# SobeyMIL/MVOC

Measured on AMD Instinct MI355X. Metric: UNet3D denoising steps/sec, 16x512^2 frames, inversion+compose, higher is better.
Workload: dtype f16

## Files before the change

mvoc_amd/csrc/pnp.hip:

```cpp
#include "common.h"

namespace {

struct PnpArgs {
  half_t* x[2];
  const half_t* masks;
  long chunk_stride, f_stride, p_stride;
  int nobj, frames, height, width, channels, mask_h, mask_w, base_chunk0;
  int ndst;
  float sy, sx;
  long total;
  int nsrc;
  unsigned obj_map;
};

template <bool MAPPED>
__device__ __forceinline__ int obj_chunk(const PnpArgs& p, int j) {
  if constexpr (MAPPED) return (int)((p.obj_map >> (4 * j)) & 15u);
  return j + 1;
}

template <bool MAPPED>
__device__ __forceinline__ int chunk_count(const PnpArgs& p) {
  if constexpr (MAPPED) return p.nsrc + p.ndst;
  return p.nobj + 1 + p.ndst;
}

__device__ __forceinline__ float blend16(float inj, float obj, float m) {
  const float om = r16(1.0f - m);
  return r16(r16(inj * om) + r16(obj * m));
}

__device__ __forceinline__ int nearest_src(int dst, float scale, int in_size) {
  return min((int)floorf(dst * scale), in_size - 1);
}

template <bool MAPPED>
__global__ __launch_bounds__(256) void pnp_tokens_kernel(const PnpArgs p) {
  const long idx = (long)blockIdx.x * 256 + threadIdx.x;
  if (idx >= p.total) return;
// ... 557 lines not shown
  MVOC_REQUIRE(d->nobj >= 1 && d->nobj <= 4, -2, "pnp: nobj %d not in [1,4]", d->nobj);
  MVOC_REQUIRE(d->frames > 0 && d->height > 0 && d->width > 0 && d->channels > 0 && d->mask_h > 0 && d->mask_w > 0, -1,
               "pnp: bad dims");
  a.x[0] = (half_t*)d->x;
  a.x[1] = (half_t*)d->x2;
  a.masks = (const half_t*)d->masks;
  a.chunk_stride = d->chunk_stride; a.f_stride = d->f_stride; a.p_stride = d->p_stride;
  a.nobj = d->nobj; a.frames = d->frames; a.height = d->height; a.width = d->width; a.channels = d->channels;
  a.mask_h = d->mask_h; a.mask_w = d->mask_w; a.base_chunk0 = d->base_chunk0;
  MVOC_REQUIRE(d->ndst >= 0 && d->ndst <= 2, -1, "pnp: ndst %d not in {0 (= 2), 1, 2}", d->ndst);
  a.ndst = d->ndst == 0 ? 2 : d->ndst;
  a.sy = (float)d->mask_h / (float)d->height;
  a.sx = (float)d->mask_w / (float)d->width;
  a.nsrc = d->nobj + 1;
  a.obj_map = 0;
  return 0;
}

int fill_map(const mvoc_pnp_desc* d, int32_t nsrc, const int32_t* obj_chunk_host, PnpArgs& a, int& nread) {
  MVOC_REQUIRE(obj_chunk_host, -1, "pnp mapped: null obj_chunk");
  MVOC_REQUIRE(nsrc >= 1 && nsrc <= d->nobj + 1, -1, "pnp mapped: nsrc %d not in [1, nobj + 1 = %d]", nsrc, d->nobj + 1);
  unsigned map = 0, seen = d->base_chunk0 ? 1u : 0u;
  for (int j = 0; j < d->nobj; ++j) {
    const int c = obj_chunk_host[j];
    MVOC_REQUIRE(c >= 0 && c < nsrc, -1, "pnp mapped: obj_chunk[%d] = %d not in [0, nsrc = %d)", j, c, nsrc);
    map |= (unsigned)c << (4 * j);
    seen |= 1u << c;
  }
  a.nsrc = nsrc;
  a.obj_map = map;
// ... 127 lines not shown
  return 0;
}

template <int NOBJ>
void launch_nchw_variants_n(bool vec, dim3 grid, hipStream_t s, const PnpArgs& a, int nvar) {
  if (vec)
    hipLaunchKernelGGL((pnp_nchw_variants_kernel<8, NOBJ>), grid, dim3(256), 0, s, a, nvar);
  else
    hipLaunchKernelGGL((pnp_nchw_variants_kernel<1, NOBJ>), grid, dim3(256), 0, s, a, nvar);
}

}

extern "C" int mvoc_pnp_blend_scatter_tokens_variants(const mvoc_pnp_desc* d, int32_t nsrc, const int32_t* obj_chunk,
                                                      int32_t nvar, void* stream) {
  PnpArgs a;
  double chunks = 0;
  if (int rc = fill_variants(d, nsrc, obj_chunk, nvar, a, chunks)) return rc;
  MVOC_REQUIRE(d->channels % 8 == 0 && d->chunk_stride % 8 == 0 && d->f_stride % 8 == 0 && d->p_stride % 8 == 0, -2,
               "pnp tokens: channels/strides must be multiples of 8");
  a.total = (long)d->frames * d->height * d->width * (d->channels / 8);
  const long nblk = (a.total + 255) / 256;
  MVOC_REQUIRE(nblk < 0x7fffffffL, -2, "pnp tokens: grid too large");
  const int ntens = d->x2 ? 2 : 1;
  hipStream_t s = (hipStream_t)stream;
  const double elems = (double)d->frames * d->height * d->width * d->channels;
  MvocProfScope prof(MVOC_FAM_PNP, s, ntens * (elems * 2.0 * chunks + 2.0 * d->nobj * d->frames * d->height * d->width));
  const dim3 grid((unsigned)nblk, ntens);
  switch (d->nobj) {
    case 1: hipLaunchKernelGGL(pnp_tokens_variants_kernel<1>, grid, dim3(256), 0, s, a, (int)nvar); break;
    case 2: hipLaunchKernelGGL(pnp_tokens_variants_kernel<2>, grid, dim3(256), 0, s, a, (int)nvar); break;
    case 3: hipLaunchKernelGGL(pnp_tokens_variants_kernel<3>, grid, dim3(256), 0, s, a, (int)nvar); break;
    default: hipLaunchKernelGGL(pnp_tokens_variants_kernel<4>, grid, dim3(256), 0, s, a, (int)nvar); break;
  }
  return mvoc_check_launch("pnp_tokens_variants_kernel");
}

extern "C" int mvoc_pnp_blend_scatter_nchw_variants(const mvoc_pnp_desc* d, int32_t nsrc, const int32_t* obj_chunk,
                                                    int32_t nvar, void* stream) {
  PnpArgs a;
  double chunks = 0;
  if (int rc = fill_variants(d, nsrc, obj_chunk, nvar, a, chunks)) return rc;
  const long hw = (long)d->height * d->width;
  const bool vec = hw % 8 == 0;
  a.total = (long)d->frames * d->channels * (vec ? hw / 8 : hw);
  const long nblk = (a.total + 255) / 256;
  MVOC_REQUIRE(nblk < 0x7fffffffL, -2, "pnp nchw: grid too large");
  const int ntens = d->x2 ? 2 : 1;
  hipStream_t s = (hipStream_t)stream;
  const double elems = (double)d->frames * hw * d->channels;
  MvocProfScope prof(MVOC_FAM_PNP, s, ntens * (elems * 2.0 * chunks + 2.0 * d->nobj * d->frames * hw));
  const dim3 grid((unsigned)nblk, ntens);
  switch (d->nobj) {
    case 1: launch_nchw_variants_n<1>(vec, grid, s, a, nvar); break;
// ... 19 lines not shown
  return 0;
}

template <int NOBJ>
void launch_nchw_variants_sel_n(bool vec, dim3 grid, hipStream_t s, const PnpArgs& a, int nvar, unsigned active) {
  if (vec)
    hipLaunchKernelGGL((pnp_nchw_variants_sel_kernel<8, NOBJ>), grid, dim3(256), 0, s, a, nvar, active);
  else
    hipLaunchKernelGGL((pnp_nchw_variants_sel_kernel<1, NOBJ>), grid, dim3(256), 0, s, a, nvar, active);
}

}

extern "C" int mvoc_pnp_blend_scatter_tokens_variants_sel(const mvoc_pnp_desc* d, int32_t nsrc, const int32_t* obj_chunk,
                                                          int32_t nvar, uint32_t active, void* stream) {
  PnpArgs a;
  double chunks = 0;
  if (int rc = fill_variants_sel(d, nsrc, obj_chunk, nvar, active, a, chunks)) return rc;
  MVOC_REQUIRE(d->channels % 8 == 0 && d->chunk_stride % 8 == 0 && d->f_stride % 8 == 0 && d->p_stride % 8 == 0, -2,
               "pnp tokens: channels/strides must be multiples of 8");
  a.total = (long)d->frames * d->height * d->width * (d->channels / 8);
  const long nblk = (a.total + 255) / 256;
  MVOC_REQUIRE(nblk < 0x7fffffffL, -2, "pnp tokens: grid too large");
  const int ntens = d->x2 ? 2 : 1;
  hipStream_t s = (hipStream_t)stream;
  const double elems = (double)d->frames * d->height * d->width * d->channels;
  MvocProfScope prof(MVOC_FAM_PNP, s, ntens * (elems * 2.0 * chunks + 2.0 * d->nobj * d->frames * d->height * d->width));
  const dim3 grid((unsigned)nblk, ntens);
  const unsigned act = active;
  switch (d->nobj) {
    case 1: hipLaunchKernelGGL(pnp_tokens_variants_sel_kernel<1>, grid, dim3(256), 0, s, a, (int)nvar, act); break;
    case 2: hipLaunchKernelGGL(pnp_tokens_variants_sel_kernel<2>, grid, dim3(256), 0, s, a, (int)nvar, act); break;
    case 3: hipLaunchKernelGGL(pnp_tokens_variants_sel_kernel<3>, grid, dim3(256), 0, s, a, (int)nvar, act); break;
    default: hipLaunchKernelGGL(pnp_tokens_variants_sel_kernel<4>, grid, dim3(256), 0, s, a, (int)nvar, act); break;
  }
  return mvoc_check_launch("pnp_tokens_variants_sel_kernel");
}

extern "C" int mvoc_pnp_blend_scatter_nchw_variants_sel(const mvoc_pnp_desc* d, int32_t nsrc, const int32_t* obj_chunk,
                                                        int32_t nvar, uint32_t active, void* stream) {
  PnpArgs a;
  double chunks = 0;
  if (int rc = fill_variants_sel(d, nsrc, obj_chunk, nvar, active, a, chunks)) return rc;
  const long hw = (long)d->height * d->width;
  const bool vec = hw % 8 == 0;
  a.total = (long)d->frames * d->channels * (vec ? hw / 8 : hw);
  const long nblk = (a.total + 255) / 256;
  MVOC_REQUIRE(nblk < 0x7fffffffL, -2, "pnp nchw: grid too large");
  const int ntens = d->x2 ? 2 : 1;
  hipStream_t s = (hipStream_t)stream;
  const double elems = (double)d->frames * hw * d->channels;
  MvocProfScope prof(MVOC_FAM_PNP, s, ntens * (elems * 2.0 * chunks + 2.0 * d->nobj * d->frames * hw));
  const dim3 grid((unsigned)nblk, ntens);
  switch (d->nobj) {
    case 1: launch_nchw_variants_sel_n<1>(vec, grid, s, a, nvar, active); break;
// ... 12 lines not shown
  return fill_variants_sel(d, nsrc, obj_chunk, nvar, active, a, chunks);
}

template <int NOBJ>
void launch_nchw_placed_n(bool vec, dim3 grid, hipStream_t s, const PnpArgs& a, int nvar, unsigned active, const int* place) {
  if (vec)
    hipLaunchKernelGGL((pnp_nchw_placed_kernel<8, NOBJ>), grid, dim3(256), 0, s, a, nvar, active, place);
  else
    hipLaunchKernelGGL((pnp_nchw_placed_kernel<1, NOBJ>), grid, dim3(256), 0, s, a, nvar, active, place);
}

}

extern "C" int mvoc_pnp_blend_scatter_tokens_placed(const mvoc_pnp_desc* d, int32_t nsrc, const int32_t* obj_chunk, int32_t nvar,
                                                    uint32_t active, const int32_t* place, void* stream) {
  PnpArgs a;
  double chunks = 0;
  if (int rc = fill_placed(d, nsrc, obj_chunk, nvar, active, place, a, chunks)) return rc;
  MVOC_REQUIRE(d->channels % 8 == 0 && d->chunk_stride % 8 == 0 && d->f_stride % 8 == 0 && d->p_stride % 8 == 0, -2,
               "pnp tokens: channels/strides must be multiples of 8");
  a.total = (long)d->frames * d->height * d->width * (d->channels / 8);
  const long nblk = (a.total + 255) / 256;
  MVOC_REQUIRE(nblk < 0x7fffffffL, -2, "pnp tokens: grid too large");
  const int ntens = d->x2 ? 2 : 1;
  hipStream_t s = (hipStream_t)stream;
  const double elems = (double)d->frames * d->height * d->width * d->channels;
  MvocProfScope prof(MVOC_FAM_PNP, s, ntens * (elems * 2.0 * chunks + 2.0 * d->nobj * d->frames * d->height * d->width));
  const dim3 grid((unsigned)nblk, ntens);
  const unsigned act = active;
  const int* pl = (const int*)place;
  switch (d->nobj) {
    case 1: hipLaunchKernelGGL(pnp_tokens_placed_kernel<1>, grid, dim3(256), 0, s, a, (int)nvar, act, pl); break;
    case 2: hipLaunchKernelGGL(pnp_tokens_placed_kernel<2>, grid, dim3(256), 0, s, a, (int)nvar, act, pl); break;
    case 3: hipLaunchKernelGGL(pnp_tokens_placed_kernel<3>, grid, dim3(256), 0, s, a, (int)nvar, act, pl); break;
    default: hipLaunchKernelGGL(pnp_tokens_placed_kernel<4>, grid, dim3(256), 0, s, a, (int)nvar, act, pl); break;
  }
  return mvoc_check_launch("pnp_tokens_placed_kernel");
}

extern "C" int mvoc_pnp_blend_scatter_nchw_placed(const mvoc_pnp_desc* d, int32_t nsrc, const int32_t* obj_chunk, int32_t nvar,
                                                  uint32_t active, const int32_t* place, void* stream) {
  PnpArgs a;
  double chunks = 0;
  if (int rc = fill_placed(d, nsrc, obj_chunk, nvar, active, place, a, chunks)) return rc;
  const long hw = (long)d->height * d->width;
  const bool vec = hw % 8 == 0;
  a.total = (long)d->frames * d->channels * (vec ? hw / 8 : hw);
  const long nblk = (a.total + 255) / 256;
  MVOC_REQUIRE(nblk < 0x7fffffffL, -2, "pnp nchw: grid too large");
  const int ntens = d->x2 ? 2 : 1;
  hipStream_t s = (hipStream_t)stream;
  const double elems = (double)d->frames * hw * d->channels;
  MvocProfScope prof(MVOC_FAM_PNP, s, ntens * (elems * 2.0 * chunks + 2.0 * d->nobj * d->frames * hw));
  const dim3 grid((unsigned)nblk, ntens);
  const int* pl = (const int*)place;
  switch (d->nobj) {
// ... 19 lines not shown
}

template <int NOBJ>
void launch_nchw_placed_variants_n(bool vec, dim3 grid, hipStream_t s, const PnpArgs& a, int nvar, unsigned active,
                                   const int* place) {
  if (vec)
    hipLaunchKernelGGL((pnp_nchw_placed_variants_kernel<8, NOBJ>), grid, dim3(256), 0, s, a, nvar, active, place);
  else
    hipLaunchKernelGGL((pnp_nchw_placed_variants_kernel<1, NOBJ>), grid, dim3(256), 0, s, a, nvar, active, place);
}

}

extern "C" int mvoc_pnp_blend_scatter_tokens_placed_variants(const mvoc_pnp_desc* d, int32_t nsrc, const int32_t* obj_chunk,
                                                             int32_t nvar, uint32_t active, const int32_t* place, void* stream) {
  PnpArgs a;
  double chunks = 0;
  int on = 0;
  if (int rc = fill_placed_variants(d, nsrc, obj_chunk, nvar, active, place, a, chunks, on)) return rc;
  MVOC_REQUIRE(d->channels % 8 == 0 && d->chunk_stride % 8 == 0 && d->f_stride % 8 == 0 && d->p_stride % 8 == 0, -2,
               "pnp tokens: channels/strides must be multiples of 8");
  a.total = (long)d->frames * d->height * d->width * (d->channels / 8);
  const long nblk = (a.total + 255) / 256;
  MVOC_REQUIRE(nblk < 0x7fffffffL, -2, "pnp tokens: grid too large");
  const int ntens = d->x2 ? 2 : 1;
  hipStream_t s = (hipStream_t)stream;
  const double elems = (double)d->frames * d->height * d->width * d->channels;
  MvocProfScope prof(MVOC_FAM_PNP, s,
                     ntens * (elems * 2.0 * chunks + 2.0 * on * d->nobj * d->frames * d->height * d->width) +
                         8.0 * nvar * d->nobj * d->frames);
  const dim3 grid((unsigned)nblk, ntens);
  const unsigned act = active;
  const int* pl = (const int*)place;
  switch (d->nobj) {
    case 1: hipLaunchKernelGGL(pnp_tokens_placed_variants_kernel<1>, grid, dim3(256), 0, s, a, (int)nvar, act, pl); break;
    case 2: hipLaunchKernelGGL(pnp_tokens_placed_variants_kernel<2>, grid, dim3(256), 0, s, a, (int)nvar, act, pl); break;
    case 3: hipLaunchKernelGGL(pnp_tokens_placed_variants_kernel<3>, grid, dim3(256), 0, s, a, (int)nvar, act, pl); break;
    default: hipLaunchKernelGGL(pnp_tokens_placed_variants_kernel<4>, grid, dim3(256), 0, s, a, (int)nvar, act, pl); break;
  }
  return mvoc_check_launch("pnp_tokens_placed_variants_kernel");
}

extern "C" int mvoc_pnp_blend_scatter_nchw_placed_variants(const mvoc_pnp_desc* d, int32_t nsrc, const int32_t* obj_chunk,
                                                           int32_t nvar, uint32_t active, const int32_t* place, void* stream) {
  PnpArgs a;
  double chunks = 0;
  int on = 0;
  if (int rc = fill_placed_variants(d, nsrc, obj_chunk, nvar, active, place, a, chunks, on)) return rc;
  const long hw = (long)d->height * d->width;
  const bool vec = hw % 8 == 0;
  a.total = (long)d->frames * d->channels * (vec ? hw / 8 : hw);
  const long nblk = (a.total + 255) / 256;
  MVOC_REQUIRE(nblk < 0x7fffffffL, -2, "pnp nchw: grid too large");
  const int ntens = d->x2 ? 2 : 1;
  hipStream_t s = (hipStream_t)stream;
  const double elems = (double)d->frames * hw * d->channels;
  MvocProfScope prof(MVOC_FAM_PNP, s,
                     ntens * (elems * 2.0 * chunks + 2.0 * on * d->nobj * d->frames * hw) + 8.0 * nvar * d->nobj * d->frames);
  const dim3 grid((unsigned)nblk, ntens);
// ... 40 lines not shown
  MVOC_REQUIRE(latents && bg && objs && masks && out && n_per > 0 && nobj >= 0, -1, "latent_fusion_variants: null operand / empty");
  MVOC_REQUIRE(nvar >= 1 && nvar <= 8, -1, "latent_fusion_variants: nvar %d not in [1, 8]", nvar);
  hipStream_t s = (hipStream_t)stream;
  const long n = (long)n_per * nvar;
  MvocProfScope prof(MVOC_FAM_MISC, s, 2.0 * n * 2 + 2.0 * n_per * (1 + 2 * nobj));
  const float mix = (float)mix_ratio, omix = (float)(1.0 - mix_ratio);
  hipLaunchKernelGGL(fusion_variants_kernel, dim3((unsigned)((n + 255) / 256)), dim3(256), 0, s, (const half_t*)latents,
                     (const half_t*)bg, (const half_t*)objs, (const half_t*)masks, (half_t*)out, nobj, (long)n_per, n, mix, omix,
                     obj_random_noise_fusion);
  return mvoc_check_launch("fusion_variants_kernel");
}

extern "C" int mvoc_pnp_blend_scatter_tokens(const mvoc_pnp_desc* d, void* stream) {
  PnpArgs a;
  if (int rc = fill_args(d, a)) return rc;
  return launch_tokens<false>(d, a, d->nobj + 1, stream);
}

extern "C" int mvoc_pnp_blend_scatter_nchw(const mvoc_pnp_desc* d, void* stream) {
  PnpArgs a;
  if (int rc = fill_args(d, a)) return rc;
  return launch_nchw<false>(d, a, d->nobj + 1, stream);
}

extern "C" int mvoc_pnp_blend_scatter_tokens_mapped(const mvoc_pnp_desc* d, int32_t nsrc, const int32_t* obj_chunk,
                                                    void* stream) {
  PnpArgs a;
  int nread = 0;
  if (int rc = fill_args(d, a)) return rc;
  if (int rc = fill_map(d, nsrc, obj_chunk, a, nread)) return rc;
  return launch_tokens<true>(d, a, nread, stream);
}

extern "C" int mvoc_pnp_blend_scatter_nchw_mapped(const mvoc_pnp_desc* d, int32_t nsrc, const int32_t* obj_chunk,
                                                  void* stream) {
  PnpArgs a;
  int nread = 0;
  if (int rc = fill_args(d, a)) return rc;
  if (int rc = fill_map(d, nsrc, obj_chunk, a, nread)) return rc;
  return launch_nchw<true>(d, a, nread, stream);
}

extern "C" int mvoc_ddim_step_f16(const void* x, const void* v_uncond, const void* v_cond, const float* coef_dev,
                                  void* out, int64_t n, void* stream) {
  MVOC_REQUIRE(x && v_cond && coef_dev && out && n > 0, -1, "ddim_step: null operand / empty");
  hipStream_t s = (hipStream_t)stream;
  MvocProfScope prof(MVOC_FAM_MISC, s, 2.0 * n * (v_uncond ? 4 : 3));
  hipLaunchKernelGGL(ddim_step_kernel, dim3((unsigned)((n + 255) / 256)), dim3(256), 0, s, (const half_t*)x,
                     (const half_t*)v_uncond, (const half_t*)v_cond, coef_dev, (half_t*)out, (long)n);
  return mvoc_check_launch("ddim_step_kernel");
// ... 15 lines not shown
```

mvoc_amd/ops.py:

```python
import ctypes as C
import os
import threading

import torch

from . import _ffi
from ._ffi import (A_CONV3X3, A_PLAIN, A_TEMPORAL3, ACT_GEGLU, ACT_GELU, ACT_NONE, ACT_SILU, AttnDesc, GemmDesc, GnDesc,
                   PnpDesc, TAttnDesc, TFusedDesc, XsDesc, check, lib)

__all__ = ["linear", "conv3x3", "tconv3", "flash_attn", "temporal_attn", "groupnorm", "groupnorm_moments", "groupnorm_apply_moments", "layernorm", "pnp_blend_tokens",
           "pnp_blend_nchw", "level_offset", "level_offsets", "place_table", "place_table_variants", "shift_planes", "ddim_step", "latent_fusion", "timestep_embedding", "act", "add", "conv3x3_small",
           "adaptive_avgpool", "ncfhw_to_tokens", "tokens_to_ncfhw", "temporal_encoder4", "conv1x1_small", "softmax_rows", "ACT_NONE", "ACT_GEGLU",
           "ACT_SILU", "ACT_GELU"]


def _stream():
    return torch.cuda.current_stream().cuda_stream


def _chk(t, name, dtype=torch.float16):
    if t is None:
        return None
    if not (isinstance(t, torch.Tensor) and t.is_cuda):
        raise RuntimeError(f"mvoc_amd.ops: `{name}` must be a device tensor (this package has no CPU path)")
# ... 20 lines not shown
USE_ROW_MOMENTS = os.environ.get("MVOC_ROW_MOMENTS", "1") != "0"


def _gemm(d: GemmDesc, dev=None, out=None, sums=False, rowmom=False):
    if dev is not None and d.act != ACT_GEGLU and d.split_k != 1:
        nbytes = lib.mvoc_gemm_workspace_bytes(d.m, d.n, d.k)
        if nbytes:
            ws = torch.empty(nbytes // 4, dtype=torch.float32, device=dev)
            d.workspace, d.workspace_bytes = ws.data_ptr(), nbytes
    cs = None
    if out is not None:
        for attr in ("chan_sums", "row_moments"):
            if hasattr(out, attr):
                delattr(out, attr)
    d.concurrency = _CONCURRENCY.n
    if sums and out is not None and d.m % 256 == 0 and d.act == ACT_NONE and out.is_contiguous() and out.shape[1] == d.n_store:
        cs = torch.empty((d.m // 256, out.shape[1], 2), dtype=torch.float32, device=out.device)
        d.chan_sums = cs.data_ptr()
    rm = None
    if rowmom and USE_ROW_MOMENTS and out is not None and d.act != ACT_GEGLU and out.is_contiguous() and out.shape[1] == d.n:
        ld = (d.n + 255) // 256
        rm = torch.empty((d.m, ld, 2), dtype=torch.float32, device=out.device)
        d.row_moments, d.row_moments_ld = rm.data_ptr(), ld
    check(lib.mvoc_gemm_f16(C.byref(d), _stream()), "gemm")
    if cs is not None and lib.mvoc_gemm_chan_sums_written():
        out.chan_sums = cs
    if rm is not None:
        w_ = lib.mvoc_gemm_row_moments_written()
        if w_:
            out.row_moments = (rm, w_)


class gemm_concurrency:

    def __init__(self, n):
        self.n = max(1, int(n))

    def __enter__(self):
        self.old, _CONCURRENCY.n = _CONCURRENCY.n, self.n
        return self
# ... 383 lines not shown
                               f"(needs {need} elements from its first)")


def _active_mask(active, nvar, what):
    if active is None:
        return None
    active, nvar = int(active), int(nvar)
    if not 1 <= nvar <= 8:
        raise RuntimeError(f"{what}: variants {nvar} not in [1, 8]")
    if not 1 <= active < (1 << nvar):
        raise RuntimeError(f"{what}: active mask {active:#x} not in [1, 2^{nvar}): bit k set = variant k injects")
    return None if active == (1 << nvar) - 1 else active


def pnp_blend_tokens(x, masks, *, frames, height, width, channels, chunk_stride, f_stride, p_stride, x2=None,
                     base_chunk0=False, ndst=2, src_map=None, nvar=1, active=None, place=None):
    d = _pnp_desc(x, x2, masks, chunk_stride, f_stride, p_stride, frames, height, width, channels, base_chunk0, ndst)
    active = _active_mask(active, nvar, "pnp_blend_tokens")
    if masks.dim() == 5 and (place is None or place.dim() != 4):
        raise RuntimeError("pnp_blend_tokens: a [K, nobj, F, mh, mw] mask stack needs place= as an int32 [K, nobj, F, 2] table")
    if nvar != 1 or place is not None:
        nsrc, chunks = _variant_map(src_map, d.nobj)
        last = (nsrc + (int(ndst) or 2) * int(nvar) - 1) * chunk_stride
        _check_variants(x, x2, nvar, last + (frames - 1) * f_stride + (height * width - 1) * p_stride + channels,
                        "pnp_blend_tokens")
        if _check_place_variants(place, masks, nvar, d.nobj, frames, "pnp_blend_tokens"):
            check(lib.mvoc_pnp_blend_scatter_tokens_placed_variants(C.byref(d), nsrc, chunks, int(nvar), _all_or(active, nvar),
                                                                    place.data_ptr(), _stream()),
                  "pnp_blend_scatter_tokens_placed_variants")
            return x
        if place is not None:
            _check_place(place, d.nobj, frames, "pnp_blend_tokens")
            check(lib.mvoc_pnp_blend_scatter_tokens_placed(C.byref(d), nsrc, chunks, int(nvar), _all_or(active, nvar),
# ... 295 lines not shown
```

mvoc_amd/pipeline.py:

```python
import hashlib
import logging
import os
import weakref
from copy import deepcopy

import torch

from . import ops
from .latent_cache import LatentCache
from .pnp_utils import register_time_all
from .schedulers import DDIMScheduler

logger = logging.getLogger(__name__)
H16 = torch.float16


class PipelineOutput:
    def __init__(self, frames=None, inverted_latents=None):
        self.frames = frames
        self.inverted_latents = inverted_latents


class SyntheticConditioner:

# ... 212 lines not shown

class I2VGenXLPipeline:

    def __init__(self, unet, scheduler=None, conditioner=None, use_graphs=True):
        self.unet = unet
        self.scheduler = scheduler or DDIMScheduler()
        self.conditioner = conditioner or SyntheticConditioner(unet.device, unet.config.cross_attention_dim)
        self.use_graphs = use_graphs
        self.vae_scale_factor = 8
        self._guidance_scale = 1.0
        self._graphs = {}
        self.max_cached_graphs = 4
        self._concurrent_states = {}
        self._streams = []
        self.prune_source_tail = os.environ.get("MVOC_PRUNE_SOURCE_TAIL", "1") != "0"
        self.share_cfg_prefix = os.environ.get("MVOC_SHARE_CFG_PREFIX", "1") != "0"
        self.dedup_sources = os.environ.get("MVOC_DEDUP_SOURCES", "0") != "0"
        self.latent_cache = LatentCache(unet.device)

    @classmethod
    def from_pretrained(cls, path, torch_dtype=H16, variant="fp16", device="cuda:0", **kw):
        import json
        from safetensors.torch import load_file
        from .unet import I2VGenXLUNet
        from .unet_spec import UNetConfig
        cfg = None
        cf = os.path.join(path, "unet", "config.json")
        if os.path.exists(cf):
            with open(cf) as fh:
                cfg = UNetConfig.from_diffusers(json.load(fh))
# ... 342 lines not shown
        prepared = self.unet.prepare_conditioning(tuple(inp.shape), mcond["fps"], mcond["image_latents_first"],
                                                  mcond["image_latents"], mcond["image_embeddings"],
                                                  mcond["encoder_hidden_states"], False)

        weak = weakref.ref(st)
        del st

        def body():
            st = weak()
            x = st["latents"]
            if do_cfg:
                inp[nb - 2 * nvar:nb - nvar].copy_(x)
            inp[nb - nvar:].copy_(x)
            u = self.unet
            saved, u.prune_source_tail = u.prune_source_tail, bool(self.prune_source_tail)
            saved_sp, u.shared_prefix_chunks = u.shared_prefix_chunks, (2 if st["share_cfg_prefix"] else 0)
            saved_sc, u.source_chunks = u.source_chunks, smap
            saved_nv, u.variants = u.variants, nvar
            saved_pl, u.placement = u.placement, st["placement"]
            saved_vp, u.variant_placements = u.variant_placements, st["variant_placements"]
            saved_vm, u.variant_masks = u.variant_masks, None if st["vplace"] is None else st["vplace"]["masks"]
            try:
                noise = u.forward_ext(inp, st["t"], mcond["fps"], mcond["image_latents_first"], mcond["image_latents"],
                                      mcond["image_embeddings"], mcond["encoder_hidden_states"], multi_frame_guidance=False,
                                      conditioning=prepared)[0]
            finally:
                u.prune_source_tail, u.shared_prefix_chunks, u.source_chunks, u.variants = saved, saved_sp, saved_sc, saved_nv
                u.placement = saved_pl
                u.variant_placements, u.variant_masks = saved_vp, saved_vm
            if st["placement"] is not None and not any(d is u._place_cache[1] for d in st["place_tables"]):
                st["place_tables"].append(u._place_cache[1])
            if st["variant_placements"] is not None and not any(d is u._vplace_cache[1] for d in st["place_tables"]):
                st["place_tables"].append(u._vplace_cache[1])
            ops.ddim_step(x, noise[nb - nvar:nb].contiguous(), st["coef"],
                          v_uncond=noise[nb - 2 * nvar:nb - nvar].contiguous() if do_cfg else None, out=x)

        return {"inp": inp, "cond": mcond, "prepared": prepared, "body": body, "nb": nb}

    def composition_step(self, st, t, bg_latents, obj_latents, table_row, fuse=None):
        if fuse is not None:
            mix, rnf, fobjs = fuse
            vp = st["vplace"]
            objs16 = [o.to(self.device, H16).contiguous() for o in fobjs] if vp is not None else None
            for k in range(st["nvar"] if vp is not None else 0):
                for j, o in enumerate(objs16):
                    ops.shift_planes(o, vp["place_dev"][k][j], out=st["fusion_objs"][j])
                lat = st["latents"][k:k + 1]
                ops.latent_fusion(lat, bg_latents, st["fusion_objs"], vp["fusion_masks"][k], mix, rnf, out=lat)
            for j, o in enumerate(fobjs if vp is None else ()):
                if st["place_dev"] is None:
                    st["fusion_objs"][j].copy_(o)
                else:
# ... 3 lines not shown
                                  nvar=st["nvar"])
            obj_latents = fobjs
        smap = plan_source_map(st.get("classes"), [bg_latents] + list(obj_latents))
        b = st["maps"].get(smap)
        if b is None:
            b = st["maps"][smap] = st["build_map"](smap)
        src = [bg_latents] + list(obj_latents)
        for c, r in enumerate(source_rows(smap, st["n_obj"])):
            b["inp"][c].copy_(src[r][0])
        st["t"].fill_(float(t))
        st["coef"].copy_(table_row)
        register_time_all(self, int(t), st["masks"])
        if not self.use_graphs:
            b["body"]()
            return
        u = self.unet
        vkey = (u.injection_masks(st["nvar"]), u.mask_key(st["masks"]), bool(u.pair_destinations), bool(u.prune_dead_chunks),
                bool(self.prune_source_tail), bool(st.get("share_cfg_prefix")), smap, st["nvar"]) + \
            (() if st["placement"] is None else (st["placement"],)) + \
            (() if st["variant_placements"] is None else ("variant_placements", st["variant_placements"]))
        g = st["variants"].get(vkey)
        if g is None:
            g = st["variants"][vkey] = GraphedStep(b["body"], preserve=(st["latents"],))
        g()

    @torch.no_grad()
    def sample_with_pnp_pipeline_with_edit_prompt_extraction_with_attn_injection(
            self, prompt=None, main_first_image=None, main_image_list=None, background_first_image=None,
            background_image_list=None, objs_first_image=None, objs_image_list=None, height=704, width=1280, target_fps=16,
            num_frames=16, num_inference_steps=50, guidance_scale=9.0, negative_prompt=None, eta=0.0,
            num_videos_per_prompt=1, decode_chunk_size=1, generator=None, latents=None, prompt_embeds=None,
            negative_prompt_embeds=None, output_type="pil", return_dict=True, cross_attention_kwargs=None, clip_skip=1,
            fusion_steps=(0, 3), ddim_init_latents_t_idx=1, ddim_inv_prompt=None, obj_mask=None, obj_width_height=None,
            obj_ddim_latents_idx_offset=None, obj_random_noise_fusion=False, random_noise_ratio=0.0,
            bg_inv_latents_path=None, obj_ddim_latents_path=None, obj_masks_tensors=None, obj_offsets=None,
# ... 154 lines not shown
```

mvoc_amd/unet.py:

```python
import math
import os
from collections import OrderedDict

import torch

from . import ops
from .ops import ACT_GEGLU, ACT_NONE, ACT_SILU
from .unet_spec import UNetConfig, param_shapes

H16 = torch.float16


def _pad_rows(w, mult=32):
    n = w.shape[0]
    if n % mult == 0:
        return w.contiguous()
    out = torch.zeros((n + mult - n % mult,) + tuple(w.shape[1:]), dtype=w.dtype, device=w.device)
    out[:n] = w
    return out


def _pad_cols(w, mult=32):
    k = w.shape[1]
    if k % mult == 0:
# ... 258 lines not shown
        h = self.proj_in.call_gn(eng, x, self.norm, nsample=nimg, rows_per_sample=hw, groups=self.groups, eps=1e-6,
                                 rowmom=True)
        c = blk.dim
        qkv = blk.attn1.to_qkv.call_ln(h, blk.norm1)
        q, k, v = qkv[:, :c], qkv[:, c:2 * c], qkv[:, 2 * c:]
        proc = blk.attn1.processor
        ndst = 0
        active = None
        if proc.injecting() and not eng._pruned:
            ndst, smap = eng.pnp_batch(B, proc.mask)
            active = eng.site_active(proc)
            masks = eng.site_masks(eng.device_masks(proc.mask)[1], 1)
            ld = qkv.stride(0)
            ops.pnp_blend_tokens(q, masks, x2=k, frames=F, height=H, width=W, channels=c, chunk_stride=F * hw * ld,
                                 f_stride=hw * ld, p_stride=ld, base_chunk0=proc.inject_background, ndst=ndst, src_map=smap,
                                 nvar=eng.variants, active=active, **eng.place_kw(proc.mask, H, W))
        if ndst == 2 and eng.pair_destinations and active is not None:
            a = torch.empty((nimg * hw, c), dtype=H16, device=x.device)
            nv = eng.variants
            ns, per = (B - 2 * nv) * F, F * hw
            s0 = slice(0, ns * hw)
            ops.flash_attn(q[s0], k[s0], v[s0], nbatch=ns, heads=self.heads, tq=hw, tk=hw, out=a[s0])
            for k0, k1, on in variant_runs(active, nv):
                su = slice(ns * hw + k0 * per, ns * hw + k1 * per)
                sc = slice(ns * hw + (nv + k0) * per, ns * hw + (nv + k1) * per)
                if on:
                    ops.flash_attn(q[su], k[su], v[su], nbatch=(k1 - k0) * F, heads=self.heads, tq=hw, tk=hw, out=a[su], v2=v[sc],
                                   out2=a[sc])
                else:
                    for sl in (su, sc):
                        ops.flash_attn(q[sl], k[sl], v[sl], nbatch=(k1 - k0) * F, heads=self.heads, tq=hw, tk=hw, out=a[sl])
# ... 49 lines not shown
            proc = attn.processor
            inject = attn is blk.attn1 and proc.injecting() and not eng._pruned
            if self.use_fused and attn.tfused is not None and not inject and F in ops.TFUSED_FRAMES and h.is_contiguous():
                a = ops.temporal_qkv_attn(h, attn.tfused, attn.to_qkv.ln, nsample=B, frames=F, hw=hw, heads=self.heads)
                h = attn.to_out(a, resid=h, rowmom=True)
                continue
            qkv = attn.to_qkv.call_ln(h, norm)
            q, k, v = qkv[:, :c], qkv[:, c:2 * c], qkv[:, 2 * c:]
            if inject:
                ndst, smap = eng.pnp_batch(B, proc.mask)
                masks = eng.site_masks(eng.section_masks(proc.mask, 0, full_hw), 0)
                ld = qkv.stride(0)
                ops.pnp_blend_tokens(q, masks, x2=k, frames=F, height=H, width=W, channels=c, chunk_stride=F * hw * ld,
                                     f_stride=hw * ld, p_stride=ld, base_chunk0=proc.inject_background, ndst=ndst,
                                     src_map=smap, nvar=eng.variants, active=eng.site_active(proc),
                                     **eng.place_kw(proc.mask, H, W))
                if eng._tail_site is self:
                    r0 = (B - ndst * eng.variants) * F * hw
                    q, k, v, h, x = q[r0:], k[r0:], v[r0:], h[r0:], x[r0:]
                    B = ndst * eng.variants
            a = ops.temporal_attn(q, k, v, nsample=B, frames=F, hw=hw, heads=self.heads)
            h = attn.to_out(a, resid=h, rowmom=True)
        f1 = blk.ff1.call_ln(h, blk.norm3, act=ACT_GEGLU)
        return self.ff_tail(blk, f1, h, x)


class ResnetBlock2D(Hookable):

    def __init__(self, sd, prefix, groups):
        super().__init__()
        g = lambda k: sd[prefix + k].to(H16).contiguous()
# ... 136 lines not shown
    def __init__(self, config=None, device="cuda:0"):
        self.config = UNetConfig.from_any(config) if config is not None else UNetConfig()
        self.device = torch.device(device)
        if self.device.type == "cuda" and torch.cuda.is_available():
            torch.cuda.set_device(self.device)
        self.dtype = H16
        self.num_upsamplers = len(self.config.block_out_channels) - 1
        self._mask_cache = (None, None, None)
        self._section_mask_cache = {}
        self._loaded = False
        self.shard = None
        self.prune_dead_chunks = True
        self._pruned = False
        self.prune_source_tail = False
        self._tail_site = None
        self.shared_prefix_chunks = 0
        self._expand_site = None
        self.pair_destinations = True
        self.source_chunks = None
        self.variants = 1
        self.placement = None
        self._place_cache = (None, {})
        self.variant_placements = None
        self.variant_masks = None
        self._vplace_cache = (None, {})

    def set_frame_shard(self, shard):
        self.shard = shard
        self.shard_generation = getattr(self, "shard_generation", 0) + 1
        self._mask_cache = (None, None, None)
# ... 107 lines not shown
                                    torch.cat([rn.time_emb_proj.b[:rn.cout] for rn in rns]))
        self._tall = None
        self._loaded = True
        self.conv_out.name, self.conv_in.name = "conv_out", "conv_in"
        named = [(f"down_blocks.{i}", b) for i, b in enumerate(self.down_blocks)] + [("mid_block", self.mid_block)]
        named += [(f"up_blocks.{i}", b) for i, b in enumerate(self.up_blocks)]
        for p, b in named:
            for kind in ("resnets", "temp_convs"):
                for j, mod in enumerate(getattr(b, kind)):
                    mod.name = f"{p}.{kind}.{j}"
            for kind in ("attentions", "temp_attentions"):
                for j, tr in enumerate(getattr(b, kind)):
                    tr.transformer_blocks[0].attn1.processor.name = f"{p}.{kind}.{j}.transformer_blocks.0.attn1.processor"

    @staticmethod
    def check_pnp_batch(B, mask_list, nsrc=None, variants=1):
        if variants != 1:
            ns = nsrc if nsrc is not None else (None if mask_list is None else len(mask_list) + 1)
            if not 1 <= variants <= 8:
                raise RuntimeError(f"variants = {variants}: 1 to 8 variants share one set of source chunks")
            if ns is None or B - ns not in (variants, 2 * variants):
                raise RuntimeError(f"PnP injection is active but the UNet batch is {B}, expected the {ns} source chunks + "
                                   f"{2 * variants} ([s.., u_1..u_{variants}, c_1..c_{variants}]) or + {variants} with guidance off")
            return (B - ns) // variants
        if nsrc is None:
            if mask_list is None or B - len(mask_list) - 1 not in (1, 2):
                raise RuntimeError(f"PnP injection is active but the UNet batch is {B}, expected n_objects+3 = "
                                   f"{None if mask_list is None else len(mask_list) + 3} ([bg, objects.., uncond, cond]) or "
                                   "n_objects+2 with guidance off; "
                                   "clear the hook state (register_time_all(pipe, None, None)) before non-composition calls")
            return B - len(mask_list) - 1
# ... 76 lines not shown
    def pnp_batch(self, B, mask_list):
        if self.placement is not None and self.shard is not None:
            raise RuntimeError("a placement does not combine with the frame shard: the section masks are cut to pixel slabs "
                               "and a shift crosses slabs")
        if self.variant_placements is not None and self.shard is not None:
            raise RuntimeError("variant_placements do not combine with the frame shard: the section masks are cut to pixel "
                               "slabs and a shift crosses slabs")
        smap = self.pnp_src_map()
        if smap is not None and len(smap[1]) != len(mask_list):
            raise RuntimeError(f"source_chunks maps {len(smap[1])} objects, the hooks carry {len(mask_list)} masks")
        if self.variants != 1:
            if self.shard is not None:
                raise RuntimeError("variants > 1 do not combine with the frame shard: run one composition per call")
            if self.shared_prefix_chunks:
                raise RuntimeError("variants > 1 do not combine with shared_prefix_chunks (DESIGN.md 6i)")
        return self.check_pnp_batch(B, mask_list, None if smap is None else smap[0], self.variants), smap

    def device_masks(self, mask_list):
        return self._all_frame_masks(mask_list)[2:]

    def _all_frame_masks(self, mask_list):
        key = self.mask_key(mask_list)
        if self._mask_cache[0] != key:
            soft = torch.stack([m[0].reshape(-1, *m[0].shape[-3:])[0] for m in mask_list]).to(self.device, H16).contiguous()
            hard = torch.stack([m[1].reshape(-1, *m[1].shape[-3:])[0] for m in mask_list]).to(self.device, H16).contiguous()
            lsoft, lhard = soft, hard
            if self.shard is not None:
                f0, f1 = self.shard.frame_range(soft.shape[1])
                lsoft, lhard = soft[:, f0:f1].contiguous(), hard[:, f0:f1].contiguous()
            keep = [(m[0], m[1]) for m in mask_list]
            self._mask_cache = (key, (soft, hard, lsoft, lhard), keep)
# ... 34 lines not shown
    def section_masks(self, mask_list, kind, full_hw):
        full = self._all_frame_masks(mask_list)[kind]
        if self.shard is None:
            return full
        key = (kind, tuple(full_hw))
        if key not in self._section_mask_cache:
            m = full
            if tuple(m.shape[2:]) != tuple(full_hw):
                m = torch.nn.functional.interpolate(m, size=tuple(full_hw), mode="nearest")
            p0, p1 = self.shard.pixel_range(full_hw[0] * full_hw[1])
            self._section_mask_cache[key] = m.reshape(m.shape[0], m.shape[1], 1, -1)[..., p0:p1].contiguous()
        return self._section_mask_cache[key]

    def inject_features(self, h, mask_list, geo, channels, full_hw=None, site=None):
        B, F, H, W = geo
        ndst, smap = self.pnp_batch(B, mask_list)
        hard = self._all_frame_masks(mask_list)[1]
        fh, fw = full_hw if full_hw is not None else (H, W)
        if hard.shape[2] != fh or hard.shape[3] != fw:
            raise RuntimeError(f"feature injection needs masks at the feature resolution {(fh, fw)}, got "
                               f"{tuple(hard.shape[2:])} (reference: pnp_utils.py:994-1000 has no resize)")
        hard = self.section_masks(mask_list, 1, full_hw) if full_hw is not None else self.device_masks(mask_list)[1]
        hard = self.site_masks(hard, 1)
        ld = h.stride(0)
        ops.pnp_blend_tokens(h, hard, frames=F, height=H, width=W, channels=channels, chunk_stride=F * H * W * ld,
                             f_stride=H * W * ld, p_stride=ld, base_chunk0=True, ndst=ndst, src_map=smap, nvar=self.variants,
                             active=None if site is None else self.site_active(site), **self.place_kw(mask_list, H, W))
        if getattr(h, "chan_sums", None) is not None:
            h.chan_sums = None

# ... 143 lines not shown
        nchw[:ns * F] = src.permute(0, 2, 1, 3, 4).reshape(ns * F, C, H, W)
        ops.pnp_blend_nchw(nchw, self.site_masks(self.device_masks(co.mask)[1], 1), frames=F, base_chunk0=True, ndst=ndst, src_map=smap,
                           nvar=self.variants, **self.place_kw(co.mask, H, W))
        return nchw.reshape(B, F, C, H, W).permute(0, 2, 1, 3, 4).contiguous()

    def spatial_transformers(self):
        for blk in list(self.down_blocks) + [self.mid_block] + list(self.up_blocks):
            yield from blk.attentions

    @torch.no_grad()
    def _forward(self, *args, **kw):
        try:
            return self._forward_impl(*args, **kw)
        finally:
            self._tall = None

    def _forward_impl(self, sample, timestep, fps, image_latents_first, image_latents, image_embeddings, encoder_hidden_states,
                      multi_frame_guidance, conditioning=None):
        if not self._loaded:
            raise RuntimeError("I2VGenXLUNet: load_state_dict() or init_random() first")
        cfg = self.config
        sample = sample.to(self.device, H16)
        B, C, F, H, W = sample.shape
        hw = H * W
        co = self.conv_out
        if self.prune_dead_chunks and not self._pruned and self.shard is None and co.injecting() and self.site_active(co) is None:
            return self._forward_source_chunks(sample, timestep, fps, image_latents_first, image_latents, image_embeddings,
                                               encoder_hidden_states, multi_frame_guidance, conditioning)
        self._tail_site = None
        if self.prune_source_tail and not self._pruned and self.shard is None and not co.injecting():
            last = self.up_blocks[-1].temp_attentions[-1] if self.up_blocks[-1].has_cross_attention else None
            if last is not None and last.transformer_blocks[0].attn1.processor.injecting():
                self._tail_site = last
        B_full = B
        up_factor = 2 ** self.num_upsamplers
        forward_upsample_size = any(s % up_factor != 0 for s in (H, W))
        temb_act = self._embeddings(timestep, fps, B)
        self._tall = self.time_proj_all(temb_act)
        sh = self.shard
        if conditioning is None:
            conditioning = self._conditioning((B, C, F, H, W), image_latents_first, image_latents, image_embeddings,
                                              encoder_hidden_states, multi_frame_guidance)
        elif conditioning.key != ((B, C, F, H, W), bool(multi_frame_guidance), id(sh)):
            raise RuntimeError(f"conditioning was prepared for {conditioning.key}, this call is "
                               f"{((B, C, F, H, W), bool(multi_frame_guidance), id(sh))}")
        ctx = conditioning.ctx
        f0, f1 = conditioning.frames

        x8 = conditioning.stem8.clone() if conditioning.key is not None else conditioning.stem8
        ops.ncfhw_to_tokens(sample, x8, coff=0)
        if sh is not None:
            x8 = x8.view(B, F, hw, 8)[:, f0:f1].reshape(-1, 8)
            F = f1 - f0
        geo = (B, F, H, W)
# ... 74 lines not shown
```

Measured before the change: 21.99.

## Prune the dead background chunk from the UNet batch when no site injects it

Adds a prune_background mode, on by default. When no injecting site blends from the background chunk (chunk 0) and the source map never references it, the forward drops that chunk from the batch: sample, embeddings, conditioning tokens and KV rows. The PnP token blend kernel gains a no_background layout in which object chunks start at index 0, and every other entry point refuses that layout. The aim is to skip a full UNet pass over one batch chunk whose outputs are never consumed, at the cost of extra layout bookkeeping and a separate graph variant key.

```diff
diff --git a/mvoc_amd/csrc/pnp.hip b/mvoc_amd/csrc/pnp.hip
--- a/mvoc_amd/csrc/pnp.hip
+++ b/mvoc_amd/csrc/pnp.hip
@@ -12,18 +12,19 @@
   long total;
   int nsrc;
   unsigned obj_map;
+  int no_background;
 };
 
 template <bool MAPPED>
 __device__ __forceinline__ int obj_chunk(const PnpArgs& p, int j) {
   if constexpr (MAPPED) return (int)((p.obj_map >> (4 * j)) & 15u);
-  return j + 1;
+  return p.no_background ? j : j + 1;
 }
 
 template <bool MAPPED>
 __device__ __forceinline__ int chunk_count(const PnpArgs& p) {
   if constexpr (MAPPED) return p.nsrc + p.ndst;
-  return p.nobj + 1 + p.ndst;
+  return p.nobj + (p.no_background ? 0 : 1) + p.ndst;
 }
 
 __device__ __forceinline__ float blend16(float inj, float obj, float m) {
@@ -611,6 +612,14 @@
   a.sx = (float)d->mask_w / (float)d->width;
   a.nsrc = d->nobj + 1;
   a.obj_map = 0;
+  a.no_background = 0;
+  return 0;
+}
+
+int refuse_no_background(const mvoc_pnp_desc* d, const char* entry) {
+  MVOC_REQUIRE(!d || d->base_chunk0 != -1, -1,
+               "%s: base_chunk0 = -1 (no background chunk) is taken by mvoc_pnp_blend_scatter_tokens only (a mapped entry expresses "
+               "the layout as nsrc = nobj, obj_chunk[j] = j; the nchw entries need chunk 0)", entry);
   return 0;
 }
 
@@ -768,6 +777,7 @@
 
 extern "C" int mvoc_pnp_blend_scatter_tokens_variants(const mvoc_pnp_desc* d, int32_t nsrc, const int32_t* obj_chunk,
                                                       int32_t nvar, void* stream) {
+  if (int rc = refuse_no_background(d, "mvoc_pnp_blend_scatter_tokens_variants")) return rc;
   PnpArgs a;
   double chunks = 0;
   if (int rc = fill_variants(d, nsrc, obj_chunk, nvar, a, chunks)) return rc;
@@ -792,6 +802,7 @@
 
 extern "C" int mvoc_pnp_blend_scatter_nchw_variants(const mvoc_pnp_desc* d, int32_t nsrc, const int32_t* obj_chunk,
                                                     int32_t nvar, void* stream) {
+  if (int rc = refuse_no_background(d, "mvoc_pnp_blend_scatter_nchw_variants")) return rc;
   PnpArgs a;
   double chunks = 0;
   if (int rc = fill_variants(d, nsrc, obj_chunk, nvar, a, chunks)) return rc;
@@ -841,6 +852,7 @@
 
 extern "C" int mvoc_pnp_blend_scatter_tokens_variants_sel(const mvoc_pnp_desc* d, int32_t nsrc, const int32_t* obj_chunk,
                                                           int32_t nvar, uint32_t active, void* stream) {
+  if (int rc = refuse_no_background(d, "mvoc_pnp_blend_scatter_tokens_variants_sel")) return rc;
   PnpArgs a;
   double chunks = 0;
   if (int rc = fill_variants_sel(d, nsrc, obj_chunk, nvar, active, a, chunks)) return rc;
@@ -866,6 +878,7 @@
 
 extern "C" int mvoc_pnp_blend_scatter_nchw_variants_sel(const mvoc_pnp_desc* d, int32_t nsrc, const int32_t* obj_chunk,
                                                         int32_t nvar, uint32_t active, void* stream) {
+  if (int rc = refuse_no_background(d, "mvoc_pnp_blend_scatter_nchw_variants_sel")) return rc;
   PnpArgs a;
   double chunks = 0;
   if (int rc = fill_variants_sel(d, nsrc, obj_chunk, nvar, active, a, chunks)) return rc;
@@ -908,6 +921,7 @@
 
 extern "C" int mvoc_pnp_blend_scatter_tokens_placed(const mvoc_pnp_desc* d, int32_t nsrc, const int32_t* obj_chunk, int32_t nvar,
                                                     uint32_t active, const int32_t* place, void* stream) {
+  if (int rc = refuse_no_background(d, "mvoc_pnp_blend_scatter_tokens_placed")) return rc;
   PnpArgs a;
   double chunks = 0;
   if (int rc = fill_placed(d, nsrc, obj_chunk, nvar, active, place, a, chunks)) return rc;
@@ -934,6 +948,7 @@
 
 extern "C" int mvoc_pnp_blend_scatter_nchw_placed(const mvoc_pnp_desc* d, int32_t nsrc, const int32_t* obj_chunk, int32_t nvar,
                                                   uint32_t active, const int32_t* place, void* stream) {
+  if (int rc = refuse_no_background(d, "mvoc_pnp_blend_scatter_nchw_placed")) return rc;
   PnpArgs a;
   double chunks = 0;
   if (int rc = fill_placed(d, nsrc, obj_chunk, nvar, active, place, a, chunks)) return rc;
@@ -983,6 +998,7 @@
 
 extern "C" int mvoc_pnp_blend_scatter_tokens_placed_variants(const mvoc_pnp_desc* d, int32_t nsrc, const int32_t* obj_chunk,
                                                              int32_t nvar, uint32_t active, const int32_t* place, void* stream) {
+  if (int rc = refuse_no_background(d, "mvoc_pnp_blend_scatter_tokens_placed_variants")) return rc;
   PnpArgs a;
   double chunks = 0;
   int on = 0;
@@ -1012,6 +1028,7 @@
 
 extern "C" int mvoc_pnp_blend_scatter_nchw_placed_variants(const mvoc_pnp_desc* d, int32_t nsrc, const int32_t* obj_chunk,
                                                            int32_t nvar, uint32_t active, const int32_t* place, void* stream) {
+  if (int rc = refuse_no_background(d, "mvoc_pnp_blend_scatter_nchw_placed_variants")) return rc;
   PnpArgs a;
   double chunks = 0;
   int on = 0;
@@ -1082,10 +1099,15 @@
 extern "C" int mvoc_pnp_blend_scatter_tokens(const mvoc_pnp_desc* d, void* stream) {
   PnpArgs a;
   if (int rc = fill_args(d, a)) return rc;
+  if (d->base_chunk0 == -1) {
+    a.no_background = 1;
+    a.base_chunk0 = 0;
+  }
   return launch_tokens<false>(d, a, d->nobj + 1, stream);
 }
 
 extern "C" int mvoc_pnp_blend_scatter_nchw(const mvoc_pnp_desc* d, void* stream) {
+  if (int rc = refuse_no_background(d, "mvoc_pnp_blend_scatter_nchw")) return rc;
   PnpArgs a;
   if (int rc = fill_args(d, a)) return rc;
   return launch_nchw<false>(d, a, d->nobj + 1, stream);
@@ -1093,6 +1115,7 @@
 
 extern "C" int mvoc_pnp_blend_scatter_tokens_mapped(const mvoc_pnp_desc* d, int32_t nsrc, const int32_t* obj_chunk,
                                                     void* stream) {
+  if (int rc = refuse_no_background(d, "mvoc_pnp_blend_scatter_tokens_mapped")) return rc;
   PnpArgs a;
   int nread = 0;
   if (int rc = fill_args(d, a)) return rc;
@@ -1102,6 +1125,7 @@
 
 extern "C" int mvoc_pnp_blend_scatter_nchw_mapped(const mvoc_pnp_desc* d, int32_t nsrc, const int32_t* obj_chunk,
                                                   void* stream) {
+  if (int rc = refuse_no_background(d, "mvoc_pnp_blend_scatter_nchw_mapped")) return rc;
   PnpArgs a;
   int nread = 0;
   if (int rc = fill_args(d, a)) return rc;
diff --git a/mvoc_amd/ops.py b/mvoc_amd/ops.py
--- a/mvoc_amd/ops.py
+++ b/mvoc_amd/ops.py
@@ -58,7 +58,8 @@
             if hasattr(out, attr):
                 delattr(out, attr)
     d.concurrency = _CONCURRENCY.n
-    if sums and out is not None and d.m % 256 == 0 and d.act == ACT_NONE and out.is_contiguous() and out.shape[1] == d.n_store:
+    want_sums = sums and out is not None and d.act == ACT_NONE and out.is_contiguous() and out.shape[1] == d.n_store
+    if want_sums and d.m % 256 == 0:
         cs = torch.empty((d.m // 256, out.shape[1], 2), dtype=torch.float32, device=out.device)
         d.chan_sums = cs.data_ptr()
     rm = None
@@ -67,7 +68,7 @@
         rm = torch.empty((d.m, ld, 2), dtype=torch.float32, device=out.device)
         d.row_moments, d.row_moments_ld = rm.data_ptr(), ld
     check(lib.mvoc_gemm_f16(C.byref(d), _stream()), "gemm")
-    if cs is not None and lib.mvoc_gemm_chan_sums_written():
+    if want_sums and lib.mvoc_gemm_chan_sums_written() and cs is not None:
         out.chan_sums = cs
     if rm is not None:
         w_ = lib.mvoc_gemm_row_moments_written()
@@ -481,9 +482,18 @@
 
 
 def pnp_blend_tokens(x, masks, *, frames, height, width, channels, chunk_stride, f_stride, p_stride, x2=None,
-                     base_chunk0=False, ndst=2, src_map=None, nvar=1, active=None, place=None):
+                     base_chunk0=False, ndst=2, src_map=None, nvar=1, active=None, place=None, no_background=False):
     d = _pnp_desc(x, x2, masks, chunk_stride, f_stride, p_stride, frames, height, width, channels, base_chunk0, ndst)
     active = _active_mask(active, nvar, "pnp_blend_tokens")
+    if no_background:
+        if base_chunk0:
+            raise RuntimeError("pnp_blend_tokens: no_background with base_chunk0: the base would be the chunk the batch does not hold")
+        if src_map is not None or nvar != 1 or place is not None or active is not None:
+            raise RuntimeError("pnp_blend_tokens: no_background is the positional entry's flag; with a source map, variants or a "
+                               "placement pass src_map=(nobj, range(nobj)) instead")
+        last = (d.nobj + (int(ndst) or 2) - 1) * chunk_stride
+        _check_variants(x, x2, 1, last + (frames - 1) * f_stride + (height * width - 1) * p_stride + channels, "pnp_blend_tokens")
+        d.base_chunk0 = -1
     if masks.dim() == 5 and (place is None or place.dim() != 4):
         raise RuntimeError("pnp_blend_tokens: a [K, nobj, F, mh, mw] mask stack needs place= as an int32 [K, nobj, F, 2] table")
     if nvar != 1 or place is not None:
diff --git a/mvoc_amd/pipeline.py b/mvoc_amd/pipeline.py
--- a/mvoc_amd/pipeline.py
+++ b/mvoc_amd/pipeline.py
@@ -250,6 +250,7 @@
         self._concurrent_states = {}
         self._streams = []
         self.prune_source_tail = os.environ.get("MVOC_PRUNE_SOURCE_TAIL", "1") != "0"
+        self.prune_background = os.environ.get("MVOC_PRUNE_BACKGROUND", "1") != "0"
         self.share_cfg_prefix = os.environ.get("MVOC_SHARE_CFG_PREFIX", "1") != "0"
         self.dedup_sources = os.environ.get("MVOC_DEDUP_SOURCES", "0") != "0"
         self.latent_cache = LatentCache(unet.device)
@@ -622,6 +623,7 @@
             inp[nb - nvar:].copy_(x)
             u = self.unet
             saved, u.prune_source_tail = u.prune_source_tail, bool(self.prune_source_tail)
+            saved_pb, u.prune_background = u.prune_background, bool(self.prune_background)
             saved_sp, u.shared_prefix_chunks = u.shared_prefix_chunks, (2 if st["share_cfg_prefix"] else 0)
             saved_sc, u.source_chunks = u.source_chunks, smap
             saved_nv, u.variants = u.variants, nvar
@@ -636,6 +638,7 @@
                 u.prune_source_tail, u.shared_prefix_chunks, u.source_chunks, u.variants = saved, saved_sp, saved_sc, saved_nv
                 u.placement = saved_pl
                 u.variant_placements, u.variant_masks = saved_vp, saved_vm
+                u.prune_background = saved_pb
             if st["placement"] is not None and not any(d is u._place_cache[1] for d in st["place_tables"]):
                 st["place_tables"].append(u._place_cache[1])
             if st["variant_placements"] is not None and not any(d is u._vplace_cache[1] for d in st["place_tables"]):
@@ -644,6 +647,23 @@
                           v_uncond=noise[nb - 2 * nvar:nb - nvar].contiguous() if do_cfg else None, out=x)
 
         return {"inp": inp, "cond": mcond, "prepared": prepared, "body": body, "nb": nb}
+
+    def background_dead(self, smap):
+        u = self.unet
+        saved = u.prune_background, u.source_chunks
+        u.prune_background, u.source_chunks = bool(self.prune_background), smap
+        try:
+            return bool(u.background_dead())
+        finally:
+            u.prune_background, u.source_chunks = saved
+
+    def composition_variant_key(self, st, smap):
+        u = self.unet
+        return (u.injection_masks(st["nvar"]), u.mask_key(st["masks"]), bool(u.pair_destinations), bool(u.prune_dead_chunks),
+                bool(self.prune_source_tail), bool(st.get("share_cfg_prefix")), smap, st["nvar"]) + \
+            (() if st["placement"] is None else (st["placement"],)) + \
+            (() if st["variant_placements"] is None else ("variant_placements", st["variant_placements"])) + \
+            (("no_background",) if self.background_dead(smap) else ())
 
     def composition_step(self, st, t, bg_latents, obj_latents, table_row, fuse=None):
         if fuse is not None:
@@ -677,11 +697,7 @@
         if not self.use_graphs:
             b["body"]()
             return
-        u = self.unet
-        vkey = (u.injection_masks(st["nvar"]), u.mask_key(st["masks"]), bool(u.pair_destinations), bool(u.prune_dead_chunks),
-                bool(self.prune_source_tail), bool(st.get("share_cfg_prefix")), smap, st["nvar"]) + \
-            (() if st["placement"] is None else (st["placement"],)) + \
-            (() if st["variant_placements"] is None else ("variant_placements", st["variant_placements"]))
+        vkey = self.composition_variant_key(st, smap)
         g = st["variants"].get(vkey)
         if g is None:
             g = st["variants"][vkey] = GraphedStep(b["body"], preserve=(st["latents"],))
diff --git a/mvoc_amd/unet.py b/mvoc_amd/unet.py
--- a/mvoc_amd/unet.py
+++ b/mvoc_amd/unet.py
@@ -296,7 +296,7 @@
             ld = qkv.stride(0)
             ops.pnp_blend_tokens(q, masks, x2=k, frames=F, height=H, width=W, channels=c, chunk_stride=F * hw * ld,
                                  f_stride=hw * ld, p_stride=ld, base_chunk0=proc.inject_background, ndst=ndst, src_map=smap,
-                                 nvar=eng.variants, active=active, **eng.place_kw(proc.mask, H, W))
+                                 nvar=eng.variants, active=active, **eng.no_background_kw(smap), **eng.place_kw(proc.mask, H, W))
         if ndst == 2 and eng.pair_destinations and active is not None:
             a = torch.empty((nimg * hw, c), dtype=H16, device=x.device)
             nv = eng.variants
@@ -376,7 +376,7 @@
                 ops.pnp_blend_tokens(q, masks, x2=k, frames=F, height=H, width=W, channels=c, chunk_stride=F * hw * ld,
                                      f_stride=hw * ld, p_stride=ld, base_chunk0=proc.inject_background, ndst=ndst,
                                      src_map=smap, nvar=eng.variants, active=eng.site_active(proc),
-                                     **eng.place_kw(proc.mask, H, W))
+                                     **eng.no_background_kw(smap), **eng.place_kw(proc.mask, H, W))
                 if eng._tail_site is self:
                     r0 = (B - ndst * eng.variants) * F * hw
                     q, k, v, h, x = q[r0:], k[r0:], v[r0:], h[r0:], x[r0:]
@@ -543,6 +543,8 @@
         self._pruned = False
         self.prune_source_tail = False
         self._tail_site = None
+        self.prune_background = False
+        self._no_bg = False
         self.shared_prefix_chunks = 0
         self._expand_site = None
         self.pair_destinations = True
@@ -680,7 +682,16 @@
                     tr.transformer_blocks[0].attn1.processor.name = f"{p}.{kind}.{j}.transformer_blocks.0.attn1.processor"
 
     @staticmethod
-    def check_pnp_batch(B, mask_list, nsrc=None, variants=1):
+    def check_pnp_batch(B, mask_list, nsrc=None, variants=1, no_background=False):
+        if no_background:
+            ns = nsrc if nsrc is not None else (None if mask_list is None else len(mask_list))
+            if not 1 <= variants <= 8:
+                raise RuntimeError(f"variants = {variants}: 1 to 8 variants share one set of source chunks")
+            if ns is None or B - ns not in (variants, 2 * variants):
+                raise RuntimeError(f"PnP injection is active but the UNet batch is {B}: without its background chunk "
+                                   f"(prune_background) the batch is the {ns} object chunks + {2 * variants} destination chunks "
+                                   f"([obj.., u_1..u_{variants}, c_1..c_{variants}]) or + {variants} with guidance off")
+            return (B - ns) // variants
         if variants != 1:
             ns = nsrc if nsrc is not None else (None if mask_list is None else len(mask_list) + 1)
             if not 1 <= variants <= 8:
@@ -787,7 +798,31 @@
                 raise RuntimeError("variants > 1 do not combine with the frame shard: run one composition per call")
             if self.shared_prefix_chunks:
                 raise RuntimeError("variants > 1 do not combine with shared_prefix_chunks (DESIGN.md 6i)")
+        if self._no_bg:
+            nsrc = (len(mask_list) if smap is None else smap[0] - 1)
+            chunks = tuple(range(nsrc)) if smap is None else tuple(c - 1 for c in smap[1])
+            ndst = self.check_pnp_batch(B, mask_list, nsrc, self.variants, no_background=True)
+            positional = smap is None and self.variants == 1 and self.placement is None and self.variant_placements is None
+            return ndst, (None if positional else (nsrc, chunks))
         return self.check_pnp_batch(B, mask_list, None if smap is None else smap[0], self.variants), smap
+
+    def no_background_kw(self, smap):
+        return {"no_background": True} if self._no_bg and smap is None else {}
+
+    def background_dead(self):
+        if not self.prune_background or self._pruned or self.shard is not None:
+            return False
+        attn = False
+        for s in self.hook_sites():
+            if not s.injecting():
+                continue
+            if not isinstance(s, Processor) or s.inject_background:
+                return False
+            attn = True
+        sc = self.source_chunks
+        if sc is not None and any(int(c) == 0 for c in sc[1]):
+            return False
+        return attn
 
     def device_masks(self, mask_list):
         return self._all_frame_masks(mask_list)[2:]
@@ -852,6 +887,7 @@
 
     def inject_features(self, h, mask_list, geo, channels, full_hw=None, site=None):
         B, F, H, W = geo
+        assert not self._no_bg, "a feature injection blends onto chunk 0: background_dead() is False on such a forward"
         ndst, smap = self.pnp_batch(B, mask_list)
         hard = self._all_frame_masks(mask_list)[1]
         fh, fw = full_hw if full_hw is not None else (H, W)
@@ -1025,6 +1061,7 @@
             return self._forward_impl(*args, **kw)
         finally:
             self._tall = None
+            self._no_bg = False
 
     def _forward_impl(self, sample, timestep, fps, image_latents_first, image_latents, image_embeddings, encoder_hidden_states,
                       multi_frame_guidance, conditioning=None):
@@ -1047,8 +1084,26 @@
         up_factor = 2 ** self.num_upsamplers
         forward_upsample_size = any(s % up_factor != 0 for s in (H, W))
         temb_act = self._embeddings(timestep, fps, B)
+        sh = self.shard
+        if conditioning is not None and conditioning.key != ((B, C, F, H, W), bool(multi_frame_guidance), id(sh)):
+            raise RuntimeError(f"conditioning was prepared for {conditioning.key}, this call is "
+                               f"{((B, C, F, H, W), bool(multi_frame_guidance), id(sh))}")
+        if self.background_dead():
+            self._no_bg = True
+            rows = lambda t: t[1:] if torch.is_tensor(t) and t.dim() > 0 and t.shape[0] == B_full else t
+            sample, temb_act = sample[1:], temb_act[1:]
+            image_latents_first, image_latents = rows(image_latents_first), rows(image_latents)
+            image_embeddings, encoder_hidden_states = rows(image_embeddings), rows(encoder_hidden_states)
+            B = B_full - 1
+            if conditioning is not None:
+                c0 = conditioning.ctx
+                per = c0.tokens.shape[0] // B_full
+                ctx = Context(c0.tokens[per:], c0.length, c0.frames_per_ctx)
+                ctx.kv = {k: v[per:] for k, v in c0.kv.items()}
+                ctx.keep = c0.keep
+                conditioning = Conditioning(ctx, conditioning.stem8[F * hw:], (B, F, H, W), conditioning.frames,
+                                            ((B, C, F, H, W), bool(multi_frame_guidance), id(sh)))
         self._tall = self.time_proj_all(temb_act)
-        sh = self.shard
         if conditioning is None:
             conditioning = self._conditioning((B, C, F, H, W), image_latents_first, image_latents, image_embeddings,
                                               encoder_hidden_states, multi_frame_guidance)
```

Measured after the change: 25.11 (median of 6 runs). 1.14x the previous value.
